# skmhrk1209/GANSynth

Measured on AMD Instinct MI355X. Metric: G+D step images/sec at 128x1024x2 mel+IF, higher is better.
Workload: dtype bf16; 1 GPU; BASELINE.json configs[1]: fully grown PGGAN 128x1024x2 G+D iteration (D update + G update, R1 + mode-seeking), per-GPU batch 8, random-init weights; global_batch=8, parallelism=dp1, launch=hipGraph replay, forked branches, forked_branches=True

## Files before the change

### gansynth_amd/_lib.py

```python
import ctypes
import os
from ctypes import c_char_p, c_double, c_float, c_int, c_int64, c_size_t, c_void_p, POINTER

_HERE = os.path.dirname(os.path.abspath(__file__))
LIB_PATH = os.path.join(_HERE, "libgansynth_hip.so")

GS_F32, GS_BF16 = 0, 1
ACT_NONE, ACT_LRELU, ACT_TANH = 0, 1, 2
ACT_LRELU_BITS, ACT_WRITE_BITS = 5, 16
PREP_CONV_FWD, PREP_CONV_BWD_DATA, PREP_CONVT_FWD, PREP_CONVT_BWD_DATA = 0, 1, 2, 3
CONV_FWD, CONV_BWD_DATA, CONV_BWD_WEIGHT = 0, 1, 2

P, I, F, L, Z = c_void_p, c_int, c_float, c_int64, c_size_t

SIGNATURES = {
    "gs_last_error": (c_char_p, []),
    "gs_version": (I, []),
    "gs_init": (I, []),
    "gs_streams_create": (I, [I, POINTER(P)]),
    "gs_streams_destroy": (I, [I, POINTER(P)]),
    "gs_prof_enable": (I, [I]),
    "gs_prof_collect": (I, [POINTER(c_int), POINTER(c_double), POINTER(c_double)]),
    "gs_prof_roofline": (I, [ctypes.c_double, ctypes.c_double, P, P, P]),
    "gs_prof_records": (I, [I, P, P, P, P, P]),
    "gs_comm_available": (I, []),
    "gs_comm_unique_id": (I, [P]),
    "gs_comm_init": (I, [POINTER(P), I, I, P]),
    "gs_comm_destroy": (I, [P]),
    "gs_comm_count": (I, [P, POINTER(I)]),
    "gs_allreduce_sum_f32": (I, [P, P, ctypes.c_int64, P]),
    "gs_comm_set_marker_us": (I, [P, ctypes.c_double]),
    "gs_broadcast_f32": (I, [P, P, ctypes.c_int64, I, P]),
    "gs_conv2d_workspace_bytes": (Z, [I, I, I, I, I, I, I, I, I]),
    "gs_conv2d_fwd": (I, [P, P, P, I, I, I, I, I, I, I, F, I, I, P, Z, P]),
    "gs_conv2d_fwd_bias_act": (I, [P, P, P, P, I, I, I, I, I, I, I, F, I, I, I, P, Z, P]),
    "gs_conv2d_bwd_data": (I, [P, P, P, I, I, I, I, I, I, I, F, I, I, P, Z, P]),
    "gs_conv2d_fwd_bias_act_norm": (I, [P, P, P, P, P, I, I, I, I, I, I, I, F, I, F, I, I, P, Z, P]),
    "gs_conv2d_transpose_s2_fwd_bias_act_norm": (I, [P, P, P, P, P, I, I, I, I, I, F, I, F, I, I, P, Z, P]),
    "gs_conv2d_fwd_mask": (I, [P, P, P, I, P, I, I, I, I, I, I, I, F, I, I, P, Z, P]),
    "gs_conv2d_bwd_data_mask": (I, [P, P, P, I, P, I, I, I, I, I, I, I, F, I, I, P, Z, P]),
    "gs_conv2d_bwd_weight": (I, [P, P, P, I, I, I, I, I, I, I, F, I, I, P, Z, P]),
    "gs_conv2d_bwd_weight_bias": (I, [P, P, P, P, I, I, I, I, I, I, I, F, I, I, P, Z, P]),
    "gs_conv2d_bwd_weight_bias_partial": (I, [P, P, P, P, I, I, I, I, I, I, I, F, I, I, P, Z, P, P]),
    "gs_conv2d_transpose_s2_bwd_weight_partial": (I, [P, P, P, I, I, I, I, I, F, I, I, P, Z, P, P]),
    "gs_wgrad_reduce_batch": (I, [P, I, P]),
    "gs_conv2d_bwd_weight_bias_multi": (I, [P, P, P, I, ctypes.c_uint, P, P, I, I, I, I, I, I, I, F, I, I, P, Z, P, P]),
    "gs_conv2d_transpose_s2_bwd_weight_multi": (I, [P, P, P, I, P, I, I, I, I, I, F, I, I, P, Z, P, P]),
    "gs_conv_wgrad_jobs_workspace_bytes": (Z, [P, I]),
    "gs_conv_wgrad_jobs": (I, [P, I, P, Z, P]),
    "gs_wgrad_cu_cap": (I, [I]),
    "gs_conv2d_transpose_s2_workspace_bytes": (Z, [I, I, I, I, I, I, I]),
    "gs_conv2d_transpose_s2_fwd": (I, [P, P, P, I, I, I, I, I, F, I, I, P, Z, P]),
    "gs_conv2d_transpose_s2_fwd_bias_act": (I, [P, P, P, P, I, I, I, I, I, F, I, I, I, P, Z, P]),
    "gs_conv2d_transpose_s2_bwd_data": (I, [P, P, P, I, I, I, I, I, F, I, I, P, Z, P]),
    "gs_conv2d_bwd_data_pnbwd_is_fused": (I, [I, I, I, I, I, I, I, I, I]),
    "gs_conv2d_fwd_pnbwdbwd_is_fused": (I, [I, I, I, I, I, I, I, I, I]),
    "gs_units_bias_act_to_nhwc": (I, [P, P, P, P, I, I, I, I, I, P]),
    "gs_nhwc_act_bwd_to_units": (I, [P, P, P, I, I, I, I, I, P]),
    "gs_conv2d_fwd_pnbwdbwd": (I, [P, P, P, P, I, F, P, P, I, I, I, I, I, I, I, F, I, I, P, Z, P]),
    "gs_conv2d_transpose_s2_fwd_pnbwdbwd": (I, [P, P, P, P, I, F, P, P, I, I, I, I, I, F, I, I, P, Z, P]),
    "gs_conv2d_bwd_data_pnbwd": (I, [P, P, P, P, I, F, P, I, I, I, I, I, I, I, F, I, I, P, Z, P]),
    "gs_conv2d_transpose_s2_bwd_data_pnbwd": (I, [P, P, P, P, I, F, P, I, I, I, I, I, F, I, I, P, Z, P]),
    "gs_conv2d_transpose_s2_bwd_weight": (I, [P, P, P, I, I, I, I, I, F, I, I, P, Z, P]),
    "gs_dense_fwd_workspace_bytes": (Z, [I, I, I]),
    "gs_dense_fwd": (I, [P, P, P, I, I, I, F, I, P, Z, P]),
    "gs_dense_fwd_bias_act": (I, [P, P, P, P, I, I, I, F, I, I, P, Z, P]),
    "gs_dense_fwd_bias_act_nhwc": (I, [P, P, P, P, I, I, I, I, F, I, I, P, Z, P]),
    "gs_dense_bwd_data": (I, [P, P, P, I, I, I, F, I, P]),
    "gs_dense_bwd_weight": (I, [P, P, P, I, I, I, F, I, I, P]),
    "gs_dense_fwd_nhwc": (I, [P, P, P, I, I, I, I, F, I, P, Z, P]),
    "gs_dense_bwd_data_nhwc": (I, [P, P, P, I, I, I, I, F, I, P]),
    "gs_dense_bwd_weight_nhwc": (I, [P, P, P, I, I, I, I, F, I, I, P]),
    "gs_embedding_fwd": (I, [P, P, P, I, I, I, F, I, P]),
    "gs_embedding_onehot_fwd": (I, [P, P, P, P, I, I, I, F, I, P]),
    "gs_embedding_bwd": (I, [P, P, P, I, I, I, F, I, P]),
    "gs_bias_act_fwd": (I, [P, P, P, L, I, I, I, P]),
    "gs_act_bwd": (I, [P, P, P, L, I, I, P]),
    "gs_act_bwd_bias": (I, [P, P, P, P, L, I, I, I, I, P, Z, P]),
    "gs_tanh_bwd_bwd": (I, [P, P, P, P, L, I, P]),
    "gs_channel_sum_workspace_bytes": (Z, [L, I]),
    "gs_channel_sum": (I, [P, P, L, I, I, I, P, Z, P]),
    "gs_bias_partial_rows": (I, [I, L, I, I]),
    "gs_channel_fold_batch_workspace_bytes": (Z, [P, I]),
# ... 99 lines not shown
```

### gansynth_amd/csrc/conv_igemm.hip

```cpp
#include <type_traits>
#include "conv_shared.h"
#include "gs_prof.h"

#ifndef GS_WGRAD_THIN_PREFETCH
#define GS_WGRAD_THIN_PREFETCH 1
#endif

extern "C" int gs_pixel_norm_fwd(const void* x, void* y, int64_t p, int c, float eps, int dtype, void* stream);
extern "C" int gs_pack_act_bits(void* z, int64_t p, int c, int dtype, void* stream);
extern "C" int gs_pixel_norm_bwd_fused(const void* g, const void* x, const void* addend, void* gx, int64_t p, int c, float eps, int pre_act, int post_act, int dtype,
                                       void* stream);
extern "C" int gs_pixel_norm_bwd_bwd_fused(const void* gg, const void* g, const void* x, void* out, void* out_g, int64_t p, int c, float eps, int pre_act,
                                           int dtype, void* stream);

namespace gs {

typedef float f32x16 __attribute__((ext_vector_type(16)));
typedef float f32x4 __attribute__((ext_vector_type(4)));
typedef __bf16 bf16x8 __attribute__((ext_vector_type(8)));


template <typename T> struct Mma;
template <> struct Mma<float> {
    typedef f32x4 frag_t;
// ... 94 lines not shown
                 : "memory", "m0");
#else
    lds_dma16(lds_addr, voff, rs);
#endif
}
__device__ __forceinline__ i32x4 make_rsrc(const void* base, unsigned bytes) {
    const unsigned long long b = reinterpret_cast<unsigned long long>(base);
    i32x4 rs;
    rs[0] = __builtin_amdgcn_readfirstlane((int)(unsigned)b);
    rs[1] = __builtin_amdgcn_readfirstlane((int)((b >> 32) & 0xffffu));
    rs[2] = __builtin_amdgcn_readfirstlane((int)bytes);
    rs[3] = 0x00020000;
    return rs;
}
__device__ __forceinline__ void wait_vmcnt(int n) {
#define GS_VM(K) case K: asm volatile("s_waitcnt vmcnt(" #K ")" ::: "memory"); break;
    switch (n) {
        GS_VM(0) GS_VM(1) GS_VM(2) GS_VM(3) GS_VM(4) GS_VM(5) GS_VM(6) GS_VM(7) GS_VM(8) GS_VM(9) GS_VM(10) GS_VM(11)
        GS_VM(12) GS_VM(13) GS_VM(14) GS_VM(15) GS_VM(16) GS_VM(17) GS_VM(18) GS_VM(19) GS_VM(20) GS_VM(21) GS_VM(22)
        GS_VM(23) GS_VM(24) GS_VM(25) GS_VM(26) GS_VM(27) GS_VM(28) GS_VM(29) GS_VM(30) GS_VM(31) GS_VM(32)
        default: asm volatile("s_waitcnt vmcnt(0)" ::: "memory"); break;
    }
#undef GS_VM
}
__device__ __forceinline__ void block_barrier() {
    asm volatile("s_waitcnt lgkmcnt(0)" ::: "memory");
    __builtin_amdgcn_s_barrier();
    asm volatile("" ::: "memory");
}

#ifndef GS_NORM_EPI_PIPELINE
#define GS_NORM_EPI_PIPELINE 1
#endif
template <typename T, int MODE, int A, int B, int TW, int TG, bool RESIDENT, int D, int NORM, int RB = 64, bool SPEC = false, bool BITS = false>
__global__ __launch_bounds__(SPEC ? 512 : 256) void conv_igemm_kernel(const ConvP p) {
    static_assert(NORM >= 0 && NORM <= 3, "NORM: 0 plain, 1 pixel norm of the result (forward blocks), 2 pixel-norm backward of the result (data gradients), "
                                          "3 both gradients of a differentiated norm backward (second-order pass)");
    constexpr int NP = 128 * B;
    constexpr int TH = NP / TW;
    constexpr int PH = patch_dim<MODE>(TH), PW = patch_dim<MODE>(TW);
    constexpr int S = MODE == MODE_S2 ? 2 : 1;
    constexpr int NPH = MODE == MODE_T2 ? 4 : 1;
    constexpr int SZ = (int)sizeof(T);
    static_assert(RB == 64 || (RB == 128 && SZ == 2), "128-byte rows: bf16 only");
    constexpr int BK = RB / SZ;
    constexpr int SL = RB / 16;
    constexpr int KS = RB / 32;
    constexpr int OCT = 32 * A;
    constexpr int NTG = 9 / TG;
    constexpr int PCH = PH * PW * SL;
    constexpr int NPP = (PCH + 63) / 64;
    constexpr int PP = (NPP + 3) / 4;
    constexpr int PBUF = PP * 4096;
    constexpr int WBYTES = TG * OCT * RB;
    constexpr int NWP = WBYTES / 1024;
    constexpr int WP = (NWP + 3) / 4;
    constexpr int WBUF = WP * 4096;
    constexpr int NPB = 1 + (D + NTG - 1) / NTG;
    constexpr int NWB = D + 1;
    constexpr int NSTEP = KS * TG;
    typedef typename Mma<T>::frag_t frag_t;

    extern __shared__ __attribute__((aligned(16))) unsigned char lds[];
    unsigned char* const lpatch = lds;
    unsigned char* const lwgt = lds + NPB * PBUF;
    float* const lbias = reinterpret_cast<float*>(lwgt + (RESIDENT ? p.nch : NWB) * WBUF);
    const unsigned a_patch = (unsigned)(uintptr_t)lds;
    const unsigned a_wgt = a_patch + NPB * PBUF;

    const T* __restrict__ wp = reinterpret_cast<const T*>(p.wp);
    T* __restrict__ y = reinterpret_cast<T*>(p.y);
    const int Hi = p.Hi, Wi = p.Wi, IC = p.IC, OC = p.OC, Hb = p.Hb, Wb = p.Wb, NCH = p.nch;

    const int tid = threadIdx.x;
    const int lane = tid & 63, hi = lane >> 5, l31 = lane & 31;
    const int wv8 = __builtin_amdgcn_readfirstlane(tid >> 6);
    const bool loader = SPEC && wv8 >= 4;
    const bool issuer = !SPEC || loader;
    const bool computer = !SPEC || !loader;
    const int wv = wv8 & 3;

    const int total = p.nsp * p.noct;
    int first, stride, count;
    if ((gridDim.x & 7) == 0) {
        const int per_xcd = (total + 7) >> 3, gx = gridDim.x >> 3;
        const int xcd = blockIdx.x & 7, loc = blockIdx.x >> 3;
        first = xcd * per_xcd + loc;
        stride = gx;
        int end = (xcd + 1) * per_xcd;
        if (end > total) end = total;
        count = first < end ? (end - first + gx - 1) / gx : 0;
    } else {
        first = blockIdx.x;
        stride = gridDim.x;
        count = first < total ? (total - first + stride - 1) / stride : 0;
    }
    if (count == 0) return;
    GS_TR(0);

    int p_voff[PP], p_lx[PP];
#pragma unroll
    for (int k = 0; k < PP; ++k) {
        const int slot = (wv + 4 * k) * 64 + lane;
        const int row = slot / SL, pos = slot % SL;
        const int ly = row / PW, lx = row - ly * PW;
        p_voff[k] = ((ly * Wi + lx) * IC) * SZ + ((pos ^ (RB == 64 ? (lx >> 2) & 3 : (lx >> 1) & 7)) << 4);
        p_lx[k] = slot < PCH ? lx : 0x40000000;
    }
    constexpr int RPP = 1024 / RB;
    constexpr int SUBS = OCT / RPP;
    const int w_lane0 = RB == 64 ? ((lane >> 2) * IC) * SZ + (((lane & 3) ^ ((lane >> 4) & 3)) << 4)
                                 : ((lane >> 3) * IC) * SZ + (((lane & 7) ^ (lane >> 4)) << 4);
    const int w_lane1 = RB == 64 ? w_lane0 : ((lane >> 3) * IC) * SZ + (((lane & 7) ^ (4 + (lane >> 4))) << 4);
    int w_soff[NTG][WP];
    bool w_odd[WP];
#pragma unroll
    for (int k = 0; k < WP; ++k) w_odd[k] = RB == 128 && (((wv + 4 * k) % SUBS) & 1);
#pragma unroll
    for (int tg = 0; tg < NTG; ++tg)
#pragma unroll
        for (int k = 0; k < WP; ++k) {
            const int j = wv + 4 * k;
            const int tt = j / SUBS, sub = j % SUBS;
            const int i = tg * TG + tt;
            const int wt = MODE == MODE_T2 ? (int)((0x453718620ULL >> (4 * (i < 9 ? i : 0))) & 15) : i;
            w_soff[tg][k] = (NWP % 4 == 0 || j < NWP) ? ((wt * OC + sub * RPP) * IC) * SZ : (int)0x80000000;
        }
    const unsigned img_bytes = (unsigned)Hi * Wi * IC * SZ;
    const unsigned w_bytes = 9u * IC * OC * SZ;
    i32x4 rs_w = make_rsrc(wp, w_bytes);
    const unsigned a_wave = wv * 1024;

    auto item_coords = [&](int item, int& n, int& by, int& bx, int& oc0) __attribute__((always_inline)) {
        const unsigned it = (unsigned)item;
        const unsigned sp = p.m_noct ? __umulhi(it, p.m_noct) : it;
        oc0 = (int)(it - sp * (unsigned)p.noct) * OCT;
        const unsigned r = p.m_tx ? __umulhi(sp, p.m_tx) : sp;
        const int tile_x = (int)(sp - r * (unsigned)p.tiles_x);
        const unsigned nn = p.m_ty ? __umulhi(r, p.m_ty) : r;
        by = (int)(r - nn * (unsigned)p.tiles_y) * TH;
        bx = tile_x * TW;
        n = (int)nn;
    };

    int i_item = first, i_left = count, i_ch = 0, i_pb = 0, i_wb = 0;
    int i_n, i_by, i_bx, i_oc0;
    item_coords(i_item, i_n, i_by, i_bx, i_oc0);
    int i_oy0 = 0, i_ox0 = 0, i_org = 0;
    i32x4 rs_x = make_rsrc(p.x, img_bytes);

    int i_wbase = 0;
    auto issue_setup = [&](int tg) __attribute__((always_inline)) {
        const bool more = i_left > 0;
        if (tg == 0) {
            i_oy0 = MODE == MODE_S2 ? 2 * i_by : i_by - 1;
            i_ox0 = MODE == MODE_S2 ? 2 * i_bx : i_bx - 1;
            i_org = ((i_oy0 * Wi + i_ox0) * IC + i_ch * BK) * SZ;
            rs_x = make_rsrc(reinterpret_cast<const unsigned char*>(p.x) + (size_t)(more ? i_n : 0) * img_bytes, more ? img_bytes : 0u);
        }
        if (!RESIDENT) {
            rs_w[2] = more ? (int)w_bytes : 0;
            i_wbase = (i_oc0 * IC + i_ch * BK) * SZ;
        }
    };
    auto issue_patch_piece = [&](int k) __attribute__((always_inline)) {
        const unsigned voff = (unsigned)(i_ox0 + p_lx[k]) < (unsigned)Wi ? (unsigned)(i_org + p_voff[k]) : 0x80000000u;
        lds_dma16(a_patch + a_wave + i_pb * PBUF + k * 4096, voff, rs_x);
    };
    auto issue_weight_piece = [&](int k, int tg, int wbase, unsigned dst_base) __attribute__((always_inline)) {
        lds_dma16_s(dst_base + a_wave + k * 4096, (unsigned)(w_odd[k] ? w_lane1 : w_lane0), rs_w, (unsigned)(w_soff[tg][k] + wbase));
    };
    constexpr int NPW = RESIDENT ? 0 : WP;
    auto stage_pieces = [](int tg) { return (tg == 0 ? PP : 0) + NPW; };
    auto issue_piece = [&](int q, int tg) __attribute__((always_inline)) {
        const int np = tg == 0 ? PP : 0;
        if (q < np) issue_patch_piece(q);
        else issue_weight_piece(q - np, tg, i_wbase, a_wgt + i_wb * WBUF);
    };
    auto issue_advance = [&](int tg) __attribute__((always_inline)) {
        if (tg == 0) i_pb = i_pb + 1 == NPB ? 0 : i_pb + 1;
        if (!RESIDENT) i_wb = i_wb + 1 == NWB ? 0 : i_wb + 1;
        if (tg == NTG - 1) {
            if (++i_ch == NCH) {
                i_ch = 0;
                --i_left;
                i_item += stride;
                if (i_left > 0) item_coords(i_item, i_n, i_by, i_bx, i_oc0);
                else i_left = 0;
            }
        }
    };

    f32x16 acc[NPH][A][B];
    auto zero_acc = [&]() __attribute__((always_inline)) {
#pragma unroll
        for (int ph = 0; ph < NPH; ++ph)
#pragma unroll
            for (int a = 0; a < A; ++a)
#pragma unroll
                for (int b = 0; b < B; ++b)
#pragma unroll
                    for (int r = 0; r < 16; ++r) acc[ph][a][b][r] = 0.f;
    };

    int b_off[B][3][KS], a_off[KS];
#pragma unroll
    for (int b = 0; b < B; ++b) {
        const int q = (wv * B + b) * 32 + l31;
        const int pb0 = ((q / TW) * S) * PW + (q % TW) * S;
#pragma unroll
        for (int ox = 0; ox < 3; ++ox) {
            const int lx = (q % TW) * S + ox;
            const int key = RB == 64 ? (lx >> 2) & 3 : (lx >> 1) & 7;
#pragma unroll
            for (int ks = 0; ks < KS; ++ks) b_off[b][ox][ks] = (pb0 + ox) * RB + (((ks * 2 + hi) ^ key) << 4);
        }
    }
#pragma unroll
    for (int ks = 0; ks < KS; ++ks) a_off[ks] = l31 * RB + (((ks * 2 + hi) ^ (RB == 64 ? (l31 >> 2) & 3 : (l31 >> 1) & 7)) << 4);

    GS_TR(1);
    if (issuer) {
        if (RESIDENT) {
            for (int ch = 0; ch < NCH; ++ch)
#pragma unroll
                for (int k = 0; k < WP; ++k) issue_weight_piece(k, 0, (i_oc0 * IC + ch * BK) * SZ, a_wgt + ch * WBUF);
        }
#pragma unroll
        for (int d = 0; d < D; ++d) {
            issue_setup(d % NTG);
#pragma unroll
            for (int q = 0; q < stage_pieces(d % NTG); ++q) issue_piece(q, d % NTG);
            issue_advance(d % NTG);
        }
    }
    GS_TR(2);
    for (int c = tid; c < OC; c += (SPEC ? 512 : 256)) lbias[c] = p.bias ? p.bias[c] : 0.f;
    zero_acc();
    if (computer) {
#pragma unroll
        for (int b = 0; b < B; ++b)
#pragma unroll
            for (int ox = 0; ox < 3; ++ox)
#pragma unroll
                for (int ks = 0; ks < KS; ++ks) asm volatile("" : "+v"(b_off[b][ox][ks]));
#pragma unroll
        for (int ks = 0; ks < KS; ++ks) asm volatile("" : "+v"(a_off[ks]));
#pragma unroll
        for (int ph = 0; ph < NPH; ++ph)
#pragma unroll
            for (int a = 0; a < A; ++a)
#pragma unroll
                for (int b = 0; b < B; ++b) asm volatile("" : "+v"(acc[ph][a][b]));
    }
    wait_vmcnt(0);
    block_barrier();
    GS_TR(3);
#ifdef GS_IGEMM_TRACE
    int tr_stage = 0;
#endif

    int item = first, done = 0, c_pb = 0, c_wb = 0;
    while (true) {
        int n, by, bx, oc0;
        item_coords(item, n, by, bx, oc0);
        unsigned mbw[BITS ? B * (MODE == MODE_T2 ? 4 : 1) : 1][A];
        constexpr bool NPIPE = (NORM == 2 || NORM == 3) && A * B <= 2 && GS_NORM_EPI_PIPELINE;
        typedef typename std::conditional<SZ == 4, float4, uint4>::type nvec_t;
        constexpr int NNV = SZ == 4 ? 4 : 2;
        nvec_t nz[NPIPE ? 2 : 1][A][NNV], nx[NPIPE ? 2 : 1][A][NNV];
// ... 1395 lines not shown
        const float v[4] = {s.x, s.y, s.z, s.w};
#pragma unroll
        for (int c = 0; c < 4; ++c) {
            float* o = q.gw + ((long)t * q.OC + oc0 + j4 + c) * q.IC + ic0 + i;
            *o = q.accumulate ? *o + v[c] * al : v[c] * al;
        }
    }
}


static int g_num_cus = 0;
static int num_cus() {
    if (g_num_cus == 0) {
        int dev = 0, n = 0;
        if (hipGetDevice(&dev) == hipSuccess && hipDeviceGetAttribute(&n, hipDeviceAttributeMultiprocessorCount, dev) == hipSuccess && n > 0)
            g_num_cus = n;
        else
            g_num_cus = 256;
    }
    return g_num_cus;
}
static int g_wgrad_cu_cap = 0;
static int wgrad_cus() {
    const int n = num_cus();
    return g_wgrad_cu_cap > 0 && g_wgrad_cu_cap < n ? g_wgrad_cu_cap : n;
}

#ifndef GS_MAX_BLOCKS_PER_CU
#define GS_MAX_BLOCKS_PER_CU 2
#endif
#ifndef GS_SMALL_D
#define GS_SMALL_D 2
#endif
template <typename T, int MODE, int A, int B, int TW, int TG, bool RESIDENT = false, int D = 2, int NORM = 0, int RB = 64, bool SPEC = false, bool BITS = false>
static int launch_igemm(ConvP p, hipStream_t st) {
    if constexpr (!BITS && sizeof(T) == 2 && NORM == 0) {
        if (p.mask_bits || p.bits_out) return launch_igemm<T, MODE, A, B, TW, TG, RESIDENT, D, NORM, RB, SPEC, true>(p, st);
    }
    constexpr int NP = 128 * B;
    constexpr int TH = NP / TW;
    constexpr int PH = patch_dim<MODE>(TH), PW = patch_dim<MODE>(TW);
    constexpr int OCT = 32 * A;
    constexpr int BK = RB / (int)sizeof(T);
    constexpr int NTG = 9 / TG;
    constexpr int PBUF = ((PH * PW * (RB / 16) + 255) / 256) * 4096;
    constexpr int WBUF = ((TG * OCT * RB + 4095) / 4096) * 4096;
    constexpr int NPB = 1 + (D + NTG - 1) / NTG, NWB = D + 1;
    p.tiles_x = cdiv(p.Wb, TW);
    p.tiles_y = cdiv(p.Hb, TH);
    p.nsp = p.N * p.tiles_x * p.tiles_y;
    p.noct = cdiv(p.OC, OCT);
    p.nch = p.IC / BK;
    {
        auto magic = [](int d) { return d <= 1 ? 0u : (unsigned)(((1ull << 32) + (unsigned)d - 1) / (unsigned)d); };
        if (p.noct >= 2048 || p.tiles_x >= 2048 || p.tiles_y >= 2048)
            return fail(GS_ERR_UNSUPPORTED, "conv igemm: %d channel tiles / %d x %d spatial tiles exceed the item decoder's range", p.noct, p.tiles_x, p.tiles_y);
        static const long max_items = getenv("GS_IGEMM_MAX_ITEMS") ? atol(getenv("GS_IGEMM_MAX_ITEMS")) : (1L << 21);
        if ((long)p.nsp * p.noct >= max_items) {
            const long per_image = (long)p.tiles_x * p.tiles_y * p.noct;
            const int chunk = (int)((max_items - 1) / per_image);
            if (chunk < 1) return fail(GS_ERR_UNSUPPORTED, "conv igemm: %ld work items per image exceed the item decoder's range", per_image);
            const size_t in_img = (size_t)p.Hi * p.Wi * p.IC * sizeof(T);
            const size_t out_img = (size_t)p.Hb * p.Wb * (MODE == MODE_T2 ? 4 : 1) * p.OC * sizeof(T);
            auto adv = [](const void* q, size_t b) -> const void* { return q ? (const char*)q + b : nullptr; };
            for (int n0 = 0; n0 < p.N; n0 += chunk) {
                ConvP q = p;
                q.N = p.N - n0 < chunk ? p.N - n0 : chunk;
                q.x = adv(p.x, n0 * in_img);
                q.y = const_cast<void*>(adv(p.y, n0 * out_img));
                q.y2 = const_cast<void*>(adv(p.y2, n0 * out_img));
                q.mask = adv(p.mask, n0 * out_img);
                q.mask_bits = reinterpret_cast<const unsigned char*>(adv(p.mask_bits, n0 * out_img / (8 * sizeof(T))));
                q.bits_out = reinterpret_cast<unsigned char*>(const_cast<void*>(adv(p.bits_out, n0 * out_img / (8 * sizeof(T)))));
                q.addend = adv(p.addend, n0 * out_img);
                int pending = 0;
                if (p.norm_pending) q.norm_pending = &pending;
                if (int e = launch_igemm<T, MODE, A, B, TW, TG, RESIDENT, D, NORM, RB, SPEC, BITS>(q, st)) return e;
                if (p.norm_pending && pending) *p.norm_pending = pending;
            }
            return 0;
        }
        p.m_noct = magic(p.noct); p.m_tx = magic(p.tiles_x); p.m_ty = magic(p.tiles_y);
    }
    const int wbufs = RESIDENT ? p.nch : NWB;
    const size_t lds = (size_t)NPB * PBUF + (size_t)wbufs * WBUF + (size_t)((p.OC + 3) / 4) * 16 + 0;
    if (p.OC % OCT != 0) return fail(GS_ERR_UNSUPPORTED, "conv igemm: %d output channels with %d-wide tiles", p.OC, OCT);
    if ((size_t)p.Hi * p.Wi * p.IC * sizeof(T) >= (1ull << 31)) return fail(GS_ERR_UNSUPPORTED, "conv igemm: one image exceeds 2 GiB");
    if (lds > 160 * 1024) return fail(GS_ERR_UNSUPPORTED, "conv igemm: %zu bytes of LDS needed", lds);
    if (NORM && p.OC != OCT) return fail(GS_ERR_UNSUPPORTED, "conv igemm: fused pixel norm needs the whole channel range in one tile");
    if ((NORM == 2 || NORM == 3) && p.OC != OCT) return fail(GS_ERR_UNSUPPORTED, "conv igemm: fused pixel-norm backward needs the whole channel range in one tile");
    if (!((NORM == 2 && p.normbwd == 1) || (NORM == 3 && p.normbwd == 2)) && p.normbwd) {
        if (p.norm_pending) *p.norm_pending = 1 + p.normbwd;
        p.normbwd = 0;
        p.mask = nullptr;
        p.addend = nullptr;
        p.y2 = nullptr;
    }
    if (NORM != 1 && NORM != 3 && p.y2) {
        if (!p.y) p.y = p.y2;
        p.y2 = nullptr;
        if (p.norm_pending) *p.norm_pending = 1;
    }
    if (p.IC % BK != 0) return fail(GS_ERR_UNSUPPORTED, "conv igemm: %d input channels with %d-channel chunks", p.IC, BK);
    auto kern = conv_igemm_kernel<T, MODE, A, B, TW, TG, RESIDENT, D, NORM, RB, SPEC, BITS>;
    static size_t max_set = 0;
    if (lds > max_set) {
        if (hipFuncSetAttribute(reinterpret_cast<const void*>(kern), hipFuncAttributeMaxDynamicSharedMemorySize, (int)lds) != hipSuccess)
            return fail(GS_ERR_HIP, "conv igemm: cannot reserve %zu bytes of dynamic LDS", lds);
        max_set = lds;
    }
    int per_cu = (int)((160 * 1024) / lds);
    if (per_cu > GS_MAX_BLOCKS_PER_CU) per_cu = GS_MAX_BLOCKS_PER_CU;
    if (per_cu < 1 || SPEC) per_cu = 1;
    const long total = (long)p.nsp * p.noct;
    long grid = (long)per_cu * num_cus();
    if (grid > total) grid = total;
    if (grid >= 8) grid &= ~7L;
    const double flops = 2.0 * 9.0 * (double)p.N * p.Hb * p.Wb * p.IC * p.OC;
    const double out_px = (double)p.N * p.Hb * p.Wb * (MODE == MODE_T2 ? 4 : 1);
    const double bytes = ((double)p.N * p.Hi * p.Wi * p.IC + out_px * p.OC * (1.0 + (p.mask ? (p.mask_bits ? 1.0 / 16.0 : 1.0) : 0.0) + (p.bits_out ? 1.0 / 16.0 : 0.0) + ((NORM == 1 && p.y) ? 1.0 : 0.0) + ((NORM == 2 && p.addend) ? 1.0 : 0.0) + (NORM == 3 ? 2.0 : 0.0)) + 9.0 * p.IC * p.OC) * sizeof(T);
    const int reps = prof_reps();
    ProfScope ps(st, flops, bytes, MODE, p.N, p.Hb, p.Wb, p.IC, p.OC, p.mask ? 1 : 0, NORM ? 1 : 0, reps);
    for (int r = 0; r < reps; ++r) hipLaunchKernelGGL(kern, dim3((unsigned)grid), dim3(SPEC ? 512 : 256), lds, st, p);
    return 0;
}

static int spec_mask() {
    static const int m = getenv("GS_SPEC") ? atoi(getenv("GS_SPEC")) : 1;
    return m;
}

template <typename T, int MODE>
static int dispatch_igemm(ConvP p, hipStream_t st) {
    constexpr int BK = 64 / (int)sizeof(T);
    const int OC = p.OC, Wb = p.Wb;
    const int nch = p.IC / BK;
    const bool resident_ok = OC == 32 && nch <= 2;
    const bool resident64_ok = OC == 64 && nch <= 2;
    const int a2 = OC % 64 == 0;
    auto items64 = [&](int B_) { return (long)p.N * cdiv(p.Hb, 4 * B_) * cdiv(Wb, 32) * (OC / 64); };
#ifdef GS_FORCE_CFG
    if constexpr (MODE == GS_FORCE_MODE && sizeof(T) == 2) return launch_igemm<T, MODE, GS_FORCE_CFG>(p, st);
#endif
    const long cus = num_cus();
    static const bool no_small = getenv("GS_NO_SMALL_TILES") != nullptr;
    const bool small = !no_small && items64(1) <= cus;
    const bool norm = p.y2 != nullptr && p.normbwd == 0;
    const bool nbwd = p.normbwd == 1;
    const bool nbb = p.normbwd == 2;
    if constexpr (MODE == MODE_T2) {
        if (resident_ok && Wb >= 64) {
            if (norm) return launch_igemm<T, MODE, 1, 1, 64, 9, true, 1, true>(p, st);
            if (nbb) return launch_igemm<T, MODE, 1, 1, 64, 9, true, 1, 3>(p, st);
            return launch_igemm<T, MODE, 1, 1, 64, 9, true, 1>(p, st);
        }
        if (small) {
            if constexpr (sizeof(T) == 2) {
                static const bool rb128 = getenv("GS_NO_RB128") == nullptr;
                if (rb128 && p.IC % 64 == 0) {
                    if (spec_mask() & 1) {
                        if (Wb >= 32) return launch_igemm<T, MODE, 1, 1, 32, 9, false, 1, false, 128, true>(p, st);
                        return launch_igemm<T, MODE, 1, 1, 16, 9, false, 1, false, 128, true>(p, st);
                    }
// ... 33 lines not shown
            if (norm) return launch_igemm<T, MODE, 1, 2, 64, 9, true, 1, true>(p, st);
            if (nbwd) return launch_igemm<T, MODE, 1, 2, 64, 9, true, 1, 2>(p, st);
            if (nbb) return launch_igemm<T, MODE, 1, 2, 64, 9, true, 1, 3>(p, st);
            return launch_igemm<T, MODE, 1, 2, 64, 9, true, 1>(p, st);
        }
        if (small) {
            if constexpr (sizeof(T) == 2) {
                static const bool rb128 = getenv("GS_NO_RB128") == nullptr;
                if (rb128 && p.IC % 64 == 0) {
                    if (spec_mask() & 1) {
                        if (Wb >= 32) return launch_igemm<T, MODE, 1, 1, 32, 9, false, 1, false, 128, true>(p, st);
                        return launch_igemm<T, MODE, 1, 1, 16, 9, false, 1, false, 128, true>(p, st);
                    }
                    if (Wb >= 32) return launch_igemm<T, MODE, 1, 1, 32, 9, false, 1, false, 128>(p, st);
                    return launch_igemm<T, MODE, 1, 1, 16, 9, false, 1, false, 128>(p, st);
                }
            }
            if (Wb >= 32) return launch_igemm<T, MODE, 1, 1, 32, 9, false, GS_SMALL_D>(p, st);
            return launch_igemm<T, MODE, 1, 1, 16, 9, false, GS_SMALL_D>(p, st);
        }
        if (!a2) return launch_igemm<T, MODE, 1, 1, 32, 3>(p, st);
        if (Wb >= 32 && items64(2) >= 2 * cus) {
            if (norm && OC == 64) return launch_igemm<T, MODE, 2, 2, 32, 3, false, 1, true>(p, st);
            if (nbwd && OC == 64) return launch_igemm<T, MODE, 2, 2, 32, 3, false, 1, 2>(p, st);
            if (nbb && OC == 64) return launch_igemm<T, MODE, 2, 2, 32, 3, false, 1, 3>(p, st);
            if (spec_mask() & 2) return launch_igemm<T, MODE, 2, 2, 32, 3, false, 2, false, 64, true>(p, st);
            return launch_igemm<T, MODE, 2, 2, 32, 3, false, 1>(p, st);
        }
        if (resident64_ok && Wb >= 32 && items64(2) >= cus / 2) return launch_igemm<T, MODE, 2, 2, 32, 9, true>(p, st);
        if (Wb >= 32 && items64(2) >= cus) {
            if (spec_mask() & 2) return launch_igemm<T, MODE, 2, 2, 32, 3, false, 2, false, 64, true>(p, st);
            if constexpr (sizeof(T) == 2) {
                static const bool rb128 = getenv("GS_NO_RB128") == nullptr;
                if (rb128 && p.IC % 64 == 0) return launch_igemm<T, MODE, 2, 2, 32, 3, false, 1, false, 128>(p, st);
            }
            return launch_igemm<T, MODE, 2, 2, 32, 3>(p, st);
        }
        if (Wb >= 32) {
            if (spec_mask() & 2) return launch_igemm<T, MODE, 2, 1, 32, 3, false, 2, false, 64, true>(p, st);
            return launch_igemm<T, MODE, 2, 1, 32, 3>(p, st);
        }
        return launch_igemm<T, MODE, 2, 1, 16, 3>(p, st);
    }
}

bool igemm_normbwd_fused(int mode, int N, int Hb, int Wb, int IC, int OC, int dtype, int form) {
    const int bk = dtype == GS_F32 ? 16 : 32;
    if (IC % bk != 0 || OC % 32 != 0) return false;
    const int nch = IC / bk;
    const long cus = num_cus();
    auto items64 = [&](int B_) { return (long)N * cdiv(Hb, 4 * B_) * cdiv(Wb, 32) * (OC / 64); };
    if (form == 2) {
        const bool small = items64(1) <= cus;
        if (mode == MODE_T2) {
            if (OC == 32 && nch <= 2 && Wb >= 64) return true;
            return !small && OC == 64 && Wb >= 32;
        }
        if (mode == MODE_S1) {
            if (OC == 32 && nch <= 2 && Wb >= 64) return true;
            return !small && OC == 64 && Wb >= 32 && items64(2) >= 2 * cus;
        }
        return false;
    }
    if (mode == MODE_S1) {
        if (OC == 32 && nch <= 2 && Wb >= 64) return true;
        const bool small = items64(1) <= cus;
        return !small && OC == 64 && Wb >= 32 && items64(2) >= 2 * cus;
// ... 271 lines not shown
        ProfScope ps(st, flops, bytes, 20 + mode, g.njobs, tw, g.nblocks, g.total_units, g.total_runs, images, 1);
#define GS_WGSK(M, TWV, SP)                                                                                              \
    do {                                                                                                                \
        constexpr int np_ = (M == MODE_S2 ? 64 : 256), th_ = np_ / TWV;                                                 \
        constexpr int lds_ = 2 * (2 * ((((patch_dim<M>(th_) * patch_dim<M>(TWV) + 15) / 16 + 3) / 4) * 4096 + np_ * 64));  \
        auto kern_ = conv_wgrad_bf16_2x2_sk_kernel<M, TWV, SP>;                                                         \
        static bool set_ = false;                                                                                       \
        if (!set_) {                                                                                                    \
            if (hipFuncSetAttribute(reinterpret_cast<const void*>(kern_), hipFuncAttributeMaxDynamicSharedMemorySize, lds_) != hipSuccess) \
                return fail(GS_ERR_HIP, "conv wgrad group: cannot reserve %d bytes of dynamic LDS", lds_);              \
            set_ = true;                                                                                                \
        }                                                                                                               \
        hipLaunchKernelGGL(kern_, dim3((unsigned)g.nblocks), dim3(SP ? 512 : 256), lds_, st, g, part);                  \
    } while (0)
        static const int spec_env = getenv("GS_SK_SPEC") ? atoi(getenv("GS_SK_SPEC")) : 0;
        const bool spec = spec_env == 1 || (spec_env == 2 && mode == MODE_S1);
        if (spec) {
            if (mode == MODE_S1) { if (tw == 32) GS_WGSK(MODE_S1, 32, true); else GS_WGSK(MODE_S1, 16, true); }
            else { if (tw == 32) GS_WGSK(MODE_S2, 32, true); else GS_WGSK(MODE_S2, 16, true); }
        } else {
            if (mode == MODE_S1) { if (tw == 32) GS_WGSK(MODE_S1, 32, false); else GS_WGSK(MODE_S1, 16, false); }
            else { if (tw == 32) GS_WGSK(MODE_S2, 32, false); else GS_WGSK(MODE_S2, 16, false); }
        }
#undef GS_WGSK
    }
    GS_CHECK_LAUNCH();
    hipLaunchKernelGGL(wgrad_sk_reduce_kernel, dim3((GS_SK_PSTRIDE / 4 + 63) / 64, (unsigned)g.total_runs), dim3(256), 0, st, g, part);
    GS_CHECK_LAUNCH();
    return 0;
}

}

extern "C" int gs_wgrad_cu_cap(int cap) {
    const int was = gs::g_wgrad_cu_cap;
    gs::g_wgrad_cu_cap = cap < 0 ? 0 : cap;
    return was;
}
extern "C" int gs_prof_enable(int on) {
    gs::g_prof.on = on != 0;
    gs::g_prof.burst = on > 1 ? on : 1;
    gs::g_prof.used = 0;
    gs::g_prof.flops = 0.0;
    return 0;
}

extern "C" int gs_prof_roofline(double peak_tflops, double peak_gbps, double* total_bytes, double* roof_ms, double* roof_ms_hbm_bound) {
    double bytes = 0.0, roof = 0.0, roof_hbm = 0.0;
    for (int i = 0; i < gs::g_prof.used; ++i) {
        if (gs::g_prof.ldesc[i][0] >= 10) continue;
        const double tf = gs::g_prof.lflops[i] / (peak_tflops * 1e12) * 1e3, tb = gs::g_prof.lbytes[i] / (peak_gbps * 1e9) * 1e3;
        bytes += gs::g_prof.lbytes[i];
        roof += tf > tb ? tf : tb;
        if (tb >= tf) roof_hbm += tb;
    }
    if (total_bytes) *total_bytes = bytes;
    if (roof_ms) *roof_ms = roof;
    if (roof_ms_hbm_bound) *roof_ms_hbm_bound = roof_hbm;
    return 0;
}

extern "C" int gs_prof_records(int max_records, int* n, double* ms, double* flops, double* bytes, int* desc) {
    int k = 0;
    for (int i = 0; i < gs::g_prof.used && k < max_records; ++i, ++k) {
        (void)hipEventSynchronize(gs::g_prof.ev[i][1]);
        float t = 0.f;
// ... 27 lines not shown
```

### include/gansynth_hip.h

```cpp
#ifndef GANSYNTH_HIP_H
#define GANSYNTH_HIP_H

#include <stddef.h>
#include <stdint.h>

#ifdef __cplusplus
extern "C" {
#endif

enum { GS_F32 = 0, GS_BF16 = 1 };
enum { GS_OK = 0, GS_ERR_ARG = -1, GS_ERR_HIP = -2, GS_ERR_UNSUPPORTED = -3, GS_ERR_WORKSPACE = -4 };
enum { GS_ACT_NONE = 0, GS_ACT_LRELU = 1, GS_ACT_TANH = 2 };
enum { GS_ACT_LRELU_BITS = 5, GS_ACT_WRITE_BITS = 16 };
enum { GS_CONV_FWD = 0, GS_CONV_BWD_DATA = 1, GS_CONV_BWD_WEIGHT = 2 };

const char* gs_last_error(void);
int gs_version(void);
int gs_init(void);
int gs_streams_create(int n, void** streams);
int gs_streams_destroy(int n, void** streams);

int gs_prof_enable(int on);
int gs_prof_collect(int* launches, double* total_ms, double* total_flops);
int gs_prof_roofline(double peak_tflops, double peak_gbps, double* total_bytes, double* roof_ms, double* roof_ms_hbm_bound);
// ... 65 lines not shown
    int32_t ic_ld;
} GsWgradReduce;
int gs_conv2d_bwd_weight_bias_partial(const void* x, const void* gy, float* gw_hwio, float* gb, int n, int h, int w, int ci, int co,
                                      int ksize, int stride, float alpha, int accumulate, int dtype, void* ws, size_t ws_bytes,
                                      GsWgradReduce* pending, void* stream);
int gs_conv2d_transpose_s2_bwd_weight_partial(const void* x, const void* gy, float* gw_hwio, int n, int h, int w, int ci, int co,
                                              float alpha, int accumulate, int dtype, void* ws, size_t ws_bytes,
                                              GsWgradReduce* pending, void* stream);
int gs_wgrad_reduce_batch(const GsWgradReduce* pending, int n, void* stream);
#define GS_WGRAD_MAX_SOURCES 4
int gs_conv2d_bwd_weight_bias_multi(const void* const* xs, const void* const* gys, const int* ns, int nsrc, unsigned bias_mask, float* gw_hwio,
                                    float* gb, int n, int h, int w, int ci, int co, int ksize, int stride, float alpha, int accumulate,
                                    int dtype, void* ws, size_t ws_bytes, GsWgradReduce* pending, void* stream);
int gs_conv2d_transpose_s2_bwd_weight_multi(const void* const* xs, const void* const* gys, const int* ns, int nsrc, float* gw_hwio, int n, int h,
                                            int w, int ci, int co, float alpha, int accumulate, int dtype, void* ws, size_t ws_bytes,
                                            GsWgradReduce* pending, void* stream);

typedef struct GsWgradJob {
    const void* x[GS_WGRAD_MAX_SOURCES];
    const void* gy[GS_WGRAD_MAX_SOURCES];
    int32_t n[GS_WGRAD_MAX_SOURCES];
    int32_t nsrc;
    uint32_t bias_mask;
    float* gw;
    float* gb;
    int32_t h, w, ci, co, ksize, stride, transposed;
    float alpha;
    int32_t accumulate, dtype;
    int32_t gw_ci_stride;
} GsWgradJob;
size_t gs_conv_wgrad_jobs_workspace_bytes(const GsWgradJob* jobs, int njobs);
int gs_conv_wgrad_jobs(const GsWgradJob* jobs, int njobs, void* ws, size_t ws_bytes, void* stream);
int gs_wgrad_cu_cap(int cap);

enum { GS_PREP_CONV_FWD = 0, GS_PREP_CONV_BWD_DATA = 1, GS_PREP_CONVT_FWD = 2, GS_PREP_CONVT_BWD_DATA = 3 };
typedef struct GsPrepDesc {
    const float* w_hwio;
    void* ws;
    int32_t map, ci, co, ksize, stride, dtype;
} GsPrepDesc;
int gs_weight_prep_batch(const GsPrepDesc* descs, int n, void* stream);

size_t gs_dense_fwd_workspace_bytes(int b, int in, int out);
int gs_dense_fwd(const void* x, const float* w, void* y, int b, int in, int out, float alpha, int dtype,
                 void* ws, size_t ws_bytes, void* stream);
int gs_dense_bwd_data(const void* gy, const float* w, void* gx, int b, int in, int out, float alpha, int dtype, void* stream);
int gs_dense_bwd_weight(const void* x, const void* gy, float* gw, int b, int in, int out, float alpha, int accumulate, int dtype,
                        void* stream);
int gs_dense_fwd_bias_act(const void* x, const float* w, const float* bias, void* y, int b, int in, int out, float alpha, int act,
                          int dtype, void* ws, size_t ws_bytes, void* stream);
int gs_dense_fwd_nhwc(const void* x, const float* w, void* y, int b, int c, int hw, int out, float alpha, int dtype,
                      void* ws, size_t ws_bytes, void* stream);
int gs_dense_fwd_bias_act_nhwc(const void* x, const float* w, const float* bias, void* y, int b, int c, int hw, int out, float alpha,
                               int act, int dtype, void* ws, size_t ws_bytes, void* stream);
int gs_dense_bwd_data_nhwc(const void* gy, const float* w, void* gx, int b, int c, int hw, int out, float alpha, int dtype, void* stream);
int gs_dense_bwd_weight_nhwc(const void* x, const void* gy, float* gw, int b, int c, int hw, int out, float alpha, int accumulate,
                             int dtype, void* stream);

int gs_embedding_fwd(const int64_t* idx, const float* w, void* y, int b, int rows, int units, float alpha, int dtype, void* stream);
int gs_embedding_onehot_fwd(const void* labels, const float* w, void* y, int64_t* idx_out, int b, int rows, int units, float alpha, int dtype, void* stream);
int gs_embedding_bwd(const int64_t* idx, const void* gy, float* gw, int b, int rows, int units, float alpha, int dtype, void* stream);

int gs_bias_act_fwd(const void* x, const float* bias, void* y, int64_t p, int c, int act, int dtype, void* stream);
int gs_act_bwd(const void* g, const void* y, void* gx, int64_t numel, int act, int dtype, void* stream);
int gs_units_bias_act_to_nhwc(const void* y, const float* bias, const void* mask, void* z, int n, int c, int hw, int act, int dtype, void* stream);
int gs_nhwc_act_bwd_to_units(const void* g, const void* z, void* gu, int n, int c, int hw, int act, int dtype, void* stream);
// ... 90 lines not shown
```

Baseline: 1658 images/sec.

## Add 8-wave conv igemm variant for RB128 bf16 path, enabled by default

Adds an NW template parameter to the implicit-GEMM conv kernel so a block can run 8 computing waves instead of 4. The patch and weight LDS buffers and the DMA piece layouts are generalized to NW. The RB128 bf16 dispatch now uses an 8-wave, B=1 configuration with one block per CU, keeping the same pixel tile while sharing LDS-staged weights across more waves. The aim is better latency hiding and fewer redundant weight loads, at the cost of less per-CU block parallelism and more register and LDS pressure per block. A C entry point can switch back to the old 4-wave variant.

```diff
diff --git a/gansynth_amd/_lib.py b/gansynth_amd/_lib.py
--- a/gansynth_amd/_lib.py
+++ b/gansynth_amd/_lib.py
@@ -49,6 +49,7 @@
     "gs_conv_wgrad_jobs_workspace_bytes": (Z, [P, I]),
     "gs_conv_wgrad_jobs": (I, [P, I, P, Z, P]),
     "gs_wgrad_cu_cap": (I, [I]),
+    "gs_igemm_test_wave_pairs": (I, [I]),
     "gs_conv2d_transpose_s2_workspace_bytes": (Z, [I, I, I, I, I, I, I]),
     "gs_conv2d_transpose_s2_fwd": (I, [P, P, P, I, I, I, I, I, F, I, I, P, Z, P]),
     "gs_conv2d_transpose_s2_fwd_bias_act": (I, [P, P, P, P, I, I, I, I, I, F, I, I, I, P, Z, P]),
diff --git a/gansynth_amd/csrc/conv_igemm.hip b/gansynth_amd/csrc/conv_igemm.hip
--- a/gansynth_amd/csrc/conv_igemm.hip
+++ b/gansynth_amd/csrc/conv_igemm.hip
@@ -150,11 +150,12 @@
 #ifndef GS_NORM_EPI_PIPELINE
 #define GS_NORM_EPI_PIPELINE 1
 #endif
-template <typename T, int MODE, int A, int B, int TW, int TG, bool RESIDENT, int D, int NORM, int RB = 64, bool SPEC = false, bool BITS = false>
-__global__ __launch_bounds__(SPEC ? 512 : 256) void conv_igemm_kernel(const ConvP p) {
+template <typename T, int MODE, int A, int B, int TW, int TG, bool RESIDENT, int D, int NORM, int RB = 64, bool SPEC = false, bool BITS = false, int NW = 4>
+__global__ __launch_bounds__(SPEC ? 512 : 64 * NW) void conv_igemm_kernel(const ConvP p) {
     static_assert(NORM >= 0 && NORM <= 3, "NORM: 0 plain, 1 pixel norm of the result (forward blocks), 2 pixel-norm backward of the result (data gradients), "
                                           "3 both gradients of a differentiated norm backward (second-order pass)");
-    constexpr int NP = 128 * B;
+    static_assert(NW == 4 || (NW == 8 && !SPEC), "NW: 4 waves, or 8 that all compute (not with loader waves)");
+    constexpr int NP = 32 * NW * B;
     constexpr int TH = NP / TW;
     constexpr int PH = patch_dim<MODE>(TH), PW = patch_dim<MODE>(TW);
     constexpr int S = MODE == MODE_S2 ? 2 : 1;
@@ -168,12 +169,12 @@
     constexpr int NTG = 9 / TG;
     constexpr int PCH = PH * PW * SL;
     constexpr int NPP = (PCH + 63) / 64;
-    constexpr int PP = (NPP + 3) / 4;
-    constexpr int PBUF = PP * 4096;
+    constexpr int PP = (NPP + NW - 1) / NW;
+    constexpr int PBUF = PP * NW * 1024;
     constexpr int WBYTES = TG * OCT * RB;
     constexpr int NWP = WBYTES / 1024;
-    constexpr int WP = (NWP + 3) / 4;
-    constexpr int WBUF = WP * 4096;
+    constexpr int WP = (NWP + NW - 1) / NW;
+    constexpr int WBUF = WP * NW * 1024;
     constexpr int NPB = 1 + (D + NTG - 1) / NTG;
     constexpr int NWB = D + 1;
     constexpr int NSTEP = KS * TG;
@@ -196,7 +197,7 @@
     const bool loader = SPEC && wv8 >= 4;
     const bool issuer = !SPEC || loader;
     const bool computer = !SPEC || !loader;
-    const int wv = wv8 & 3;
+    const int wv = NW == 8 ? wv8 : wv8 & 3;
 
     const int total = p.nsp * p.noct;
     int first, stride, count;
@@ -219,7 +220,7 @@
     int p_voff[PP], p_lx[PP];
 #pragma unroll
     for (int k = 0; k < PP; ++k) {
-        const int slot = (wv + 4 * k) * 64 + lane;
+        const int slot = (wv + NW * k) * 64 + lane;
         const int row = slot / SL, pos = slot % SL;
         const int ly = row / PW, lx = row - ly * PW;
         p_voff[k] = ((ly * Wi + lx) * IC) * SZ + ((pos ^ (RB == 64 ? (lx >> 2) & 3 : (lx >> 1) & 7)) << 4);
@@ -233,16 +234,16 @@
     int w_soff[NTG][WP];
     bool w_odd[WP];
 #pragma unroll
-    for (int k = 0; k < WP; ++k) w_odd[k] = RB == 128 && (((wv + 4 * k) % SUBS) & 1);
+    for (int k = 0; k < WP; ++k) w_odd[k] = RB == 128 && (((wv + NW * k) % SUBS) & 1);
 #pragma unroll
     for (int tg = 0; tg < NTG; ++tg)
 #pragma unroll
         for (int k = 0; k < WP; ++k) {
-            const int j = wv + 4 * k;
+            const int j = wv + NW * k;
             const int tt = j / SUBS, sub = j % SUBS;
             const int i = tg * TG + tt;
             const int wt = MODE == MODE_T2 ? (int)((0x453718620ULL >> (4 * (i < 9 ? i : 0))) & 15) : i;
-            w_soff[tg][k] = (NWP % 4 == 0 || j < NWP) ? ((wt * OC + sub * RPP) * IC) * SZ : (int)0x80000000;
+            w_soff[tg][k] = (NWP % NW == 0 || j < NWP) ? ((wt * OC + sub * RPP) * IC) * SZ : (int)0x80000000;
         }
     const unsigned img_bytes = (unsigned)Hi * Wi * IC * SZ;
     const unsigned w_bytes = 9u * IC * OC * SZ;
@@ -283,10 +284,10 @@
     };
     auto issue_patch_piece = [&](int k) __attribute__((always_inline)) {
         const unsigned voff = (unsigned)(i_ox0 + p_lx[k]) < (unsigned)Wi ? (unsigned)(i_org + p_voff[k]) : 0x80000000u;
-        lds_dma16(a_patch + a_wave + i_pb * PBUF + k * 4096, voff, rs_x);
+        lds_dma16(a_patch + a_wave + i_pb * PBUF + k * (NW * 1024), voff, rs_x);
     };
     auto issue_weight_piece = [&](int k, int tg, int wbase, unsigned dst_base) __attribute__((always_inline)) {
-        lds_dma16_s(dst_base + a_wave + k * 4096, (unsigned)(w_odd[k] ? w_lane1 : w_lane0), rs_w, (unsigned)(w_soff[tg][k] + wbase));
+        lds_dma16_s(dst_base + a_wave + k * (NW * 1024), (unsigned)(w_odd[k] ? w_lane1 : w_lane0), rs_w, (unsigned)(w_soff[tg][k] + wbase));
     };
     constexpr int NPW = RESIDENT ? 0 : WP;
     auto stage_pieces = [](int tg) { return (tg == 0 ? PP : 0) + NPW; };
@@ -353,7 +354,7 @@
         }
     }
     GS_TR(2);
-    for (int c = tid; c < OC; c += (SPEC ? 512 : 256)) lbias[c] = p.bias ? p.bias[c] : 0.f;
+    for (int c = tid; c < OC; c += (SPEC ? 512 : 64 * NW)) lbias[c] = p.bias ? p.bias[c] : 0.f;
     zero_acc();
     if (computer) {
 #pragma unroll
@@ -1815,19 +1816,19 @@
 #ifndef GS_SMALL_D
 #define GS_SMALL_D 2
 #endif
-template <typename T, int MODE, int A, int B, int TW, int TG, bool RESIDENT = false, int D = 2, int NORM = 0, int RB = 64, bool SPEC = false, bool BITS = false>
+template <typename T, int MODE, int A, int B, int TW, int TG, bool RESIDENT = false, int D = 2, int NORM = 0, int RB = 64, bool SPEC = false, bool BITS = false, int NW = 4>
 static int launch_igemm(ConvP p, hipStream_t st) {
     if constexpr (!BITS && sizeof(T) == 2 && NORM == 0) {
-        if (p.mask_bits || p.bits_out) return launch_igemm<T, MODE, A, B, TW, TG, RESIDENT, D, NORM, RB, SPEC, true>(p, st);
-    }
-    constexpr int NP = 128 * B;
+        if (p.mask_bits || p.bits_out) return launch_igemm<T, MODE, A, B, TW, TG, RESIDENT, D, NORM, RB, SPEC, true, NW>(p, st);
+    }
+    constexpr int NP = 32 * NW * B;
     constexpr int TH = NP / TW;
     constexpr int PH = patch_dim<MODE>(TH), PW = patch_dim<MODE>(TW);
     constexpr int OCT = 32 * A;
     constexpr int BK = RB / (int)sizeof(T);
     constexpr int NTG = 9 / TG;
-    constexpr int PBUF = ((PH * PW * (RB / 16) + 255) / 256) * 4096;
-    constexpr int WBUF = ((TG * OCT * RB + 4095) / 4096) * 4096;
+    constexpr int PBUF = ((PH * PW * (RB / 16) + 64 * NW - 1) / (64 * NW)) * (NW * 1024);
+    constexpr int WBUF = ((TG * OCT * RB + NW * 1024 - 1) / (NW * 1024)) * (NW * 1024);
     constexpr int NPB = 1 + (D + NTG - 1) / NTG, NWB = D + 1;
     p.tiles_x = cdiv(p.Wb, TW);
     p.tiles_y = cdiv(p.Hb, TH);
@@ -1858,7 +1859,7 @@
                 q.addend = adv(p.addend, n0 * out_img);
                 int pending = 0;
                 if (p.norm_pending) q.norm_pending = &pending;
-                if (int e = launch_igemm<T, MODE, A, B, TW, TG, RESIDENT, D, NORM, RB, SPEC, BITS>(q, st)) return e;
+                if (int e = launch_igemm<T, MODE, A, B, TW, TG, RESIDENT, D, NORM, RB, SPEC, BITS, NW>(q, st)) return e;
                 if (p.norm_pending && pending) *p.norm_pending = pending;
             }
             return 0;
@@ -1885,7 +1886,7 @@
         if (p.norm_pending) *p.norm_pending = 1;
     }
     if (p.IC % BK != 0) return fail(GS_ERR_UNSUPPORTED, "conv igemm: %d input channels with %d-channel chunks", p.IC, BK);
-    auto kern = conv_igemm_kernel<T, MODE, A, B, TW, TG, RESIDENT, D, NORM, RB, SPEC, BITS>;
+    auto kern = conv_igemm_kernel<T, MODE, A, B, TW, TG, RESIDENT, D, NORM, RB, SPEC, BITS, NW>;
     static size_t max_set = 0;
     if (lds > max_set) {
         if (hipFuncSetAttribute(reinterpret_cast<const void*>(kern), hipFuncAttributeMaxDynamicSharedMemorySize, (int)lds) != hipSuccess)
@@ -1894,7 +1895,7 @@
     }
     int per_cu = (int)((160 * 1024) / lds);
     if (per_cu > GS_MAX_BLOCKS_PER_CU) per_cu = GS_MAX_BLOCKS_PER_CU;
-    if (per_cu < 1 || SPEC) per_cu = 1;
+    if (per_cu < 1 || SPEC || NW == 8) per_cu = 1;
     const long total = (long)p.nsp * p.noct;
     long grid = (long)per_cu * num_cus();
     if (grid > total) grid = total;
@@ -1904,7 +1905,7 @@
     const double bytes = ((double)p.N * p.Hi * p.Wi * p.IC + out_px * p.OC * (1.0 + (p.mask ? (p.mask_bits ? 1.0 / 16.0 : 1.0) : 0.0) + (p.bits_out ? 1.0 / 16.0 : 0.0) + ((NORM == 1 && p.y) ? 1.0 : 0.0) + ((NORM == 2 && p.addend) ? 1.0 : 0.0) + (NORM == 3 ? 2.0 : 0.0)) + 9.0 * p.IC * p.OC) * sizeof(T);
     const int reps = prof_reps();
     ProfScope ps(st, flops, bytes, MODE, p.N, p.Hb, p.Wb, p.IC, p.OC, p.mask ? 1 : 0, NORM ? 1 : 0, reps);
-    for (int r = 0; r < reps; ++r) hipLaunchKernelGGL(kern, dim3((unsigned)grid), dim3(SPEC ? 512 : 256), lds, st, p);
+    for (int r = 0; r < reps; ++r) hipLaunchKernelGGL(kern, dim3((unsigned)grid), dim3(SPEC ? 512 : 64 * NW), lds, st, p);
     return 0;
 }
 
@@ -1912,6 +1913,8 @@
     static const int m = getenv("GS_SPEC") ? atoi(getenv("GS_SPEC")) : 1;
     return m;
 }
+
+static int g_igemm_wave_pairs = 1;
 
 template <typename T, int MODE>
 static int dispatch_igemm(ConvP p, hipStream_t st) {
@@ -2011,7 +2014,10 @@
             if (spec_mask() & 2) return launch_igemm<T, MODE, 2, 2, 32, 3, false, 2, false, 64, true>(p, st);
             if constexpr (sizeof(T) == 2) {
                 static const bool rb128 = getenv("GS_NO_RB128") == nullptr;
-                if (rb128 && p.IC % 64 == 0) return launch_igemm<T, MODE, 2, 2, 32, 3, false, 1, false, 128>(p, st);
+                if (rb128 && p.IC % 64 == 0) {
+                    if (g_igemm_wave_pairs) return launch_igemm<T, MODE, 2, 1, 32, 3, false, 1, false, 128, false, false, 8>(p, st);
+                    return launch_igemm<T, MODE, 2, 2, 32, 3, false, 1, false, 128>(p, st);
+                }
             }
             return launch_igemm<T, MODE, 2, 2, 32, 3>(p, st);
         }
@@ -2349,6 +2355,11 @@
 
 }
 
+extern "C" int gs_igemm_test_wave_pairs(int mask) {
+    const int was = gs::g_igemm_wave_pairs;
+    gs::g_igemm_wave_pairs = mask != 0;
+    return was;
+}
 extern "C" int gs_wgrad_cu_cap(int cap) {
     const int was = gs::g_wgrad_cu_cap;
     gs::g_wgrad_cu_cap = cap < 0 ? 0 : cap;
diff --git a/include/gansynth_hip.h b/include/gansynth_hip.h
--- a/include/gansynth_hip.h
+++ b/include/gansynth_hip.h
@@ -121,6 +121,7 @@
 size_t gs_conv_wgrad_jobs_workspace_bytes(const GsWgradJob* jobs, int njobs);
 int gs_conv_wgrad_jobs(const GsWgradJob* jobs, int njobs, void* ws, size_t ws_bytes, void* stream);
 int gs_wgrad_cu_cap(int cap);
+int gs_igemm_test_wave_pairs(int mask);
 
 enum { GS_PREP_CONV_FWD = 0, GS_PREP_CONV_BWD_DATA = 1, GS_PREP_CONVT_FWD = 2, GS_PREP_CONVT_BWD_DATA = 3 };
 typedef struct GsPrepDesc {
```

Result: no change. 1668 images/sec (median of 2 runs) (+0.6%).
